# jing2li/MGPreconditionedGCR

Hardware: AMD Instinct MI355X
Metric: gcr_iterations_per_sec (higher is better)
Workload: dtype f64; 1 GPU; 3D 7-point Poisson 128^3 per GPU, unpreconditioned GCR restart 5, complex fp64, x0=0, RHS splitmix64 seed 0; rows=2097152, nnz=14581760, complex=True, stored_matrix_bytes=2097292, ell_width=7, tail_nnz=0, partition=1 GPU

## Files before the change

mgpreconditionedgcr_amd/csrc/gcr.hip:

```cpp
#include <climits>
#include <cmath>
#include <type_traits>

#include "internal.h"
#include "reduce.h"
#include "gcr_dev.h"
#include "pw_tail_dev.h"

namespace mgcr {

static EnvSwitch g_lean{"MGCR_LEAN"};
bool set_lean_enabled(bool on) { return g_lean.set(on); }

static double g_prof_phase_ms[3] = {0., 0., 0.};
static int g_prof_iters = 0;
static int g_prof_fused = 0;
void gcr_last_profile(double *phase_ms_total, int *n_iter, int *fused) {
    for (int k = 0; k < 3; k++) phase_ms_total[k] = g_prof_phase_ms[k];
    *n_iter = g_prof_iters;
    *fused = g_prof_fused;
}

struct GcrState {
    Op *A = nullptr;
// ... 1028 lines not shown
    s->r_after.clear();
    if (!p.left_precond && (!p.right_precond || pl.flex) && pl.max_it <= LND) s->r_after.assign((size_t)pl.max_it + 1, nullptr);
    return MGCR_OK;
}

struct Step {
    int it;
    bool tail;
    int lim;
    int ic_next;
    int nxt;
    const cplx *dir = nullptr;
    bool xr_now = false;
    const cplx *xr_in = nullptr;
    bool ended = false;
};

static int step_residual_lean(GcrState *s, const SolvePlan &pl, StepCursor &c, Step &st) {
    const int cur = c.cur;
    cplx *dslot = st.nxt >= 1 ? s->ps[st.nxt] : (pl.flex ? s->z : s->r);
    cplx *r_out = pl.flex ? s->r : dslot;
    const bool alpha_only = st.tail && pl.nested && !pl.multi;
    const bool deferred = alpha_only && s->defer_residual && !pl.flex && !s->r_after.empty();
    if (deferred || (alpha_only && s->discard_residual)) {
        KLAUNCH(alpha_only_kernel, 1, s->st, st.it, c.refA.p, c.refA.nblk, c.refA.stride, s->den + cur, cur, s->lc,
                deferred ? s->alphas + cur : (cplx *)nullptr);
        if (deferred) {
            s->defer_r_prev = c.rcur; s->defer_ap = s->aps[cur]; s->defer_alpha = s->alphas + cur; s->defer_it = c.global;
            s->r_after[(size_t)c.global] = c.rcur;
        } else {
            s->r_after.clear();
        }
        st.ended = true;
        return MGCR_OK;
    }
    st.xr_now = pl.xr_fuse && !st.tail;
    st.xr_in = c.rcur;
    if (c.xr_prefetched) c.xr_prefetched = false;
    else if (!st.xr_now)
        KLAUNCH((xr_update_kernel<true, true>), pl.g, s->st, st.it, c.refA.p, c.refA.nblk, c.refA.stride, (const cplx *)nullptr,
                (const cplx *)s->aps[cur], pl.x, c.rcur, r_out, pl.n, s->partsR, s->den + cur, s->alphas, cur, s->lc);
    c.rcur = r_out;
    st.dir = r_out;
    if (pl.flex && !st.tail) {
        MGCR_TRY(op_apply_raw((Op *)s->p.right_precond, s->r, dslot, pl.n));
        st.dir = dslot;
    }
    return MGCR_OK;
}

static int step_residual_classic(GcrState *s, const SolvePlan &pl, StepCursor &c, Step &st) {
    const mgcr_gcr_param &p = s->p;
    const int cur = c.cur;
// ... 34 lines not shown
static int step_one_launch(GcrState *s, const SolvePlan &pl, StepCursor &c, PhaseMarks &marks, const Step &st) {
    const int lim = st.lim;
    const bool closes = st.ic_next == 0;
    const cplx *vecs[FND], *cps[FND];
    for (int j = 0; j < FND; j++) { vecs[j] = s->aps[j < lim ? j : 0]; cps[j] = j < lim && j > 0 ? s->ps[j] : c.p0_live; }
    cplx *xr_out = nullptr;
    const bool next_is_special_last = c.global + 1 == pl.max_it && pl.nested && (s->defer_residual || s->discard_residual);
    if (c.global + 1 <= pl.max_it && !next_is_special_last && g_stepbuild_xr.on()) {
        const int ic2 = ((st.ic_next + 1) % s->restart == 0) ? 0 : st.ic_next + 1;
        const int nxt2 = ic2 % s->storage;
        MGCR_TRY(ensure_slot(s, nxt2));
        xr_out = nxt2 >= 1 ? s->ps[nxt2] : s->r;
    }
    MGCR_TRY(csr_step_build(pl.b0->csr, st.dir, pl.shift, pl.k, vecs, lim, s->st, st.it, c.refR.p, c.refR.nblk, c.refR.stride, s->hist,
                            s->hist_cap, s->den, s->aps[st.nxt], s->partsA, s->lc, pl.rmap, xr_out, s->den + st.nxt, st.nxt, s->partsR,
                            closes ? cps : nullptr, closes ? s->ps[0] : nullptr, closes ? pl.x : nullptr));
    c.xr_prefetched = xr_out != nullptr;
    marks.step_build = true;
    marks.step_build_xr = marks.step_build_xr || c.xr_prefetched;
    marks.step_build_close = marks.step_build_close || closes;
    if (closes) c.p0_live = s->ps[0];
    return MGCR_OK;
}

static int step_apply_dots(GcrState *s, const SolvePlan &pl, const StepCursor &c, const Step &st, bool *tail_rb) {
    const int lim = st.lim, nchunk = (lim + ND - 1) / ND;
    int ch0 = 0;
    if (pl.fuse_ok) {
        const int nf = lim < FND ? lim : FND;
        const cplx *vecs[FND];
        for (int j = 0; j < FND; j++) vecs[j] = s->aps[j < nf ? j : 0];
// ... 317 lines not shown
```

mgpreconditionedgcr_amd/csrc/gcr_dev.h:

```cpp
#pragma once
#include "internal.h"
#include "reduce.h"
#include "fused_form.h"

namespace mgcr {

constexpr int ND = 8;
constexpr int FND = 10;
constexpr int LND = 16;
#ifndef MGCR_NT_SLOTS
#define MGCR_NT_SLOTS 1
#endif
constexpr bool NTS = MGCR_NT_SLOTS != 0;

struct DevState {
    int stop_at;
    int base;
    int iter;
    int npend;
    double bnorm2;
    double rr;
    double tol2;
    int closed;
};
// ... 150 lines not shown
    }
    return c;
}

bool gcr_resident_eligible(const Op *A, const mgcr_gcr_param &p, int storage, int restart, int64_t n, bool lean, bool nested_handoff);
int gcr_resident_run(Op *A, const mgcr_gcr_param &p, int storage, int restart, const cplx *rhs, cplx *x, bool from_zero, bool alpha_only_last,
                     DevState *st, double *hist, int hist_cap, cplx *ring , SkipRef outer);

bool csr_step_build_eligible(const CsrDev &A, const DistCsr *dist, int lim);
bool csr_start_build_eligible(const CsrDev &A, const DistCsr *dist);
int csr_start_build(const CsrDev &A, const cplx *b, bool shift, cplx k, cplx *ap0, DevState *st, double *hist, LeanCoef *lc, cplx *den0,
                    cplx *r_out, double *partsR_out, const RowMap &rm);
int csr_step_build(const CsrDev &A, const cplx *x, bool shift, cplx k, const cplx *const *aps, int nd, DevState *st, int it, const double *partsR,
                   int nblkR, int strideR, double *hist, int hist_cap, const cplx *den, cplx *ap_out, double *partsA, LeanCoef *lc,
                   const RowMap &rm, cplx *xr_out = nullptr, cplx *xr_den_slot = nullptr, int xr_slot = 0, double *partsR_out = nullptr,
                   const cplx *const *close_ps = nullptr, cplx *close_p_out = nullptr, cplx *close_x = nullptr);

}
```

mgpreconditionedgcr_amd/csrc/gcr_stepbuild.hip:

```cpp
#include <climits>
#include <cstdlib>
#include <type_traits>

#include "internal.h"
#include "reduce.h"
#include "gcr_dev.h"
#include "spmv_dev.h"
#include "exchange_dev.h"

namespace mgcr {

constexpr int SB_MAX_TRIPS = 4;
constexpr int SB_MAX_ND = 5;
constexpr int SB_KEEP_TB = 2;
template <int NDT> constexpr int sb_keep_rows() { return NDT == 1 ? 3 : 2; }
template <int NDT, bool XR, bool CLOSE> constexpr bool sb_close_merged() { return CLOSE && (NDT == 4 || (NDT == 5 && XR)); }

struct StepBuildArgs {
    RowMat m;
    const cplx *x;
    const cplx *aps[SB_MAX_ND];
    int64_t n;
    int nlogical;
    RowMap rm;
    DevState *st;
    int it;
    const double *partsR;
    int nblkR, strideR;
    double *hist;
    int hist_cap;
    const cplx *den;
    cplx *ap_out;
    double *partsA;
    LeanCoef *lc;
    const cplx *ps[SB_MAX_ND];
    cplx *p_out;
    cplx *xvec;
    cplx *xr_out;
    cplx *xr_den_slot;
    int xr_slot;
    double *partsR_out;
    v4i *slots;
    unsigned gen0;
    unsigned *abort_dev;
    int *abort_host;
    int spin_limit;
    int test_stall;
};

__device__ __forceinline__ cplx sb_xr_alpha(const ResSync &sy, DevState *st, LeanCoef *lc, cplx *xr_den_slot, int xr_slot, int lb) {
    const cplx num = make_double2(res_total(sy, 0), res_total(sy, 1)), den = make_double2(res_total(sy, 2), res_total(sy, 3));
    const cplx alpha = to_sgpr(cdiv(num, den));
    if (lb == 0 && threadIdx.x == 0) {
        *xr_den_slot = den;
        st->npend = xr_slot + 1;
    }
    if (lb == 0 && (int)threadIdx.x < LND) lean_pending_update(lc, xr_slot, alpha, (int)threadIdx.x);
    return alpha;
}

template <int MODE, int WT, int NDT, bool XR, bool CLOSE, bool REALC = false>
__global__ void __launch_bounds__(RED_THREADS, 8) step_build_kernel(StepBuildArgs a) {
    __shared__ double lds[(2 * NDT > 4 ? 2 * NDT : 4) * 17];
    __shared__ double lds_pw[2 * SB_MAX_ND * 17], lds_ws[2 * SB_MAX_ND * RES_GRP];
    __shared__ int gave_up;
    __shared__ cplx sbeta[NDT], scp[NDT];
    extern __shared__ __attribute__((aligned(16))) unsigned char sb_smem[];
    if (a.st->stop_at < a.st->base + a.it) return;
    const int lb = logical_workgroup(a.rm, (int)blockIdx.x, (int)gridDim.x);
    if (lb >= a.nlogical) return;
    cplx *arL = reinterpret_cast<cplx *>(sb_smem);
    ResSync sy;
    res_sync_init(sy, a.slots, a.gen0, a.nlogical, lb, a.abort_dev, a.spin_limit, lds_pw, lds_ws, &gave_up);
    if (a.test_stall && lb == a.test_stall - 1) return;
    int64_t i0, end, stride;
    row_range(a.rm, lb, a.nlogical, a.n, &i0, &end, &stride);
    {
        double v[2 * NDT];
#pragma unroll
        for (int j = 0; j < 2 * NDT; j++) v[j] = 0.;
        int trip = 0;
        for (int64_t i = i0; i < end; i += stride, trip++) {
            const PatLds pl{nullptr, nullptr, nullptr};
            cplx sum;
            if constexpr (REALC) sum = sten_row_product_t<WT, false, 1>(a.m, i, [&](int32_t j) -> cplx { return a.x[j]; });
            else sum = fused_row_product<MODE, WT>(a.m, i, 0, pl, [&](int32_t j) -> cplx { return a.x[j]; });
            const cplx yi = a.m.shift ? csub(a.x[i], cmul(a.m.k, sum)) : sum;
            arL[trip * RED_THREADS + (int)threadIdx.x] = yi;
            __builtin_amdgcn_sched_barrier(0);
            cplx b[NDT];
#pragma unroll
            for (int j = 0; j < NDT; j++) b[j] = ld_stream<true>(a.aps[j] + i);
#pragma unroll
            for (int j = 0; j < NDT; j++) {
                cplx t = cconj_mul(yi, b[j]);
                v[2 * j] += t.x;
                v[2 * j + 1] += t.y;
            }
        }
        const double mine = block_sum_owner<2 * NDT>(v, lds);
        if ((int)threadIdx.x < 2 * NDT) {
            const v4i w4 = {__double2loint(mine), __double2hiint(mine), (int)sy.gen, 0};
            __builtin_amdgcn_raw_buffer_store_b128(w4, sy.slots, ((1 * RES_NV + (int)threadIdx.x) * RES_BLK + lb) * 16, 0, RES_SC1);
        }
    }
    constexpr bool PRE = NDT <= 3;
    cplx pre[NDT];
#pragma unroll
    for (int j = 0; j < NDT; j++) pre[j] = make_double2(0., 0.);
    if (PRE && i0 < end) {
#pragma unroll
        for (int j = 0; j < NDT; j++) pre[j] = ld_stream<NTS>((CLOSE ? a.ps[j] : a.aps[j]) + i0);
    }
    const bool ok = res_collect<2 * NDT>(sy, 1);
    if (!ok) {
        res_abort(a.abort_dev, a.abort_host);
        for (int64_t i = i0; i < end; i += stride) a.ap_out[i] = make_double2(__builtin_nan(""), __builtin_nan(""));
        if ((int)threadIdx.x < 4) a.partsA[threadIdx.x * RED_MAX_BLOCKS + lb] = __builtin_nan("");
        return;
    }
    bool ends_here = false;
    if (XR || lb == 0) {
        double rr[1];
        fold_partials<1>(a.partsR, a.nblkR, a.strideR, rr, lds);
        if (lb == 0 && threadIdx.x == 0) {
            close_step(a.st, a.it, rr[0], a.hist, a.hist_cap, CLOSE);
            if (CLOSE) a.st->closed = 1;
        }
        ends_here = !((rr[0] / a.st->bnorm2) > a.st->tol2);
    }
    if ((int)threadIdx.x < NDT) sbeta[threadIdx.x] = cdiv(make_double2(res_total(sy, 2 * threadIdx.x), res_total(sy, 2 * threadIdx.x + 1)), a.den[threadIdx.x]);
    __syncthreads();
    if constexpr (CLOSE) {
        if ((int)threadIdx.x < NDT) scp[threadIdx.x] = lean_close_coef(a.lc, sbeta, NDT, (int)threadIdx.x);
        __syncthreads();
    }
    if (!CLOSE && lb == 0 && (int)threadIdx.x <= NDT) lean_table_row<NDT>(a.lc, sbeta, (int)threadIdx.x);
    cplx beta[NDT];
#pragma unroll
    for (int j = 0; j < NDT; j++) beta[j] = to_sgpr(sbeta[j]);
    double v[4] = {0., 0., 0., 0.};
    int trip = 0;
    constexpr bool MERGED = sb_close_merged<NDT, XR, CLOSE>();
    cplx mcp[MERGED ? NDT : 1], mcx[MERGED ? NDT : 1];
    if constexpr (MERGED) {
#pragma unroll
        for (int j = 0; j < NDT; j++) {
            mcp[j] = to_sgpr(scp[j]);
            mcx[j] = to_sgpr(a.lc->cx[j]);
        }
    }
    auto close_row = [&](int64_t i, cplx dv) {
        cplx pj[NDT];
#pragma unroll
        for (int j = 0; j < NDT; j++) pj[j] = ld_stream<NTS>(a.ps[j] + i);
        cplx xv = a.xvec[i];
#pragma unroll
        for (int j = 0; j < NDT; j++) xv = cadd(xv, cmul(mcx[MERGED ? j : 0], pj[j]));
        a.xvec[i] = xv;
        cplx pc = make_double2(0., 0.);
#pragma unroll
        for (int j = 0; j < NDT; j++) pc = csub(pc, cmul(mcp[MERGED ? j : 0], pj[j]));
        st_stream<NTS>(a.p_out + i, cadd(dv, pc));
    };
    if constexpr (CLOSE && !MERGED) {
        cplx cp[NDT], cx[NDT];
#pragma unroll
        for (int j = 0; j < NDT; j++) {
            cp[j] = to_sgpr(scp[j]);
            cx[j] = to_sgpr(a.lc->cx[j]);
        }
        for (int64_t i = i0; i < end; i += stride) {
            cplx pj[NDT];
#pragma unroll
            for (int j = 0; j < NDT; j++) pj[j] = (PRE && i == i0) ? pre[j] : ld_stream<NTS>(a.ps[j] + i);
            const cplx dv = a.x[i];
            cplx xv = a.xvec[i];
#pragma unroll
            for (int j = 0; j < NDT; j++) xv = cadd(xv, cmul(cx[j], pj[j]));
            a.xvec[i] = xv;
            cplx pc = make_double2(0., 0.);
#pragma unroll
            for (int j = 0; j < NDT; j++) pc = csub(pc, cmul(cp[j], pj[j]));
            st_stream<NTS>(a.p_out + i, cadd(dv, pc));
        }
// ... 15 lines not shown
        cplx u = cconj_mul(an, an);
        v[2] += u.x; v[3] += u.y;
        return rv;
    };
    if constexpr (MERGED) {
        for (int64_t i = i0; i < end; i += stride, trip++) {
            const cplx rv = a.x[i];
            if (!XR || i + stride < end) close_row(i, rv);
            __builtin_amdgcn_sched_barrier(0);
            (void)build_row(i, trip, rv);
            __builtin_amdgcn_sched_barrier(0);
        }
    } else {
        for (int64_t i = i0; i < end; i += stride, trip++) (void)build_row(i, trip, make_double2(0., 0.));
    }
    const double mine = block_sum_owner<4>(v, lds);
    if (threadIdx.x < 4) a.partsA[threadIdx.x * RED_MAX_BLOCKS + lb] = mine;
    auto close_last = [&]() {
        if (trip > 0) {
            const int64_t il = i0 + (int64_t)(trip - 1) * stride;
            close_row(il, a.x[il]);
        }
        __builtin_amdgcn_sched_barrier(0);
    };
    if constexpr (XR) {
        if ((int)threadIdx.x < 4) {
            const v4i w4 = {__double2loint(mine), __double2hiint(mine), (int)sy.gen, 0};
            __builtin_amdgcn_raw_buffer_store_b128(w4, sy.slots, ((2 * RES_NV + (int)threadIdx.x) * RES_BLK + lb) * 16, 0, RES_SC1);
        }
        if constexpr (MERGED) close_last();
        const cplx xr0 = i0 < end ? a.x[i0] : make_double2(0., 0.);
        if (!res_collect<4>(sy, 2)) {
            res_abort(a.abort_dev, a.abort_host);
            for (int64_t i = i0; i < end; i += stride) a.xr_out[i] = make_double2(__builtin_nan(""), __builtin_nan(""));
            if (threadIdx.x == 0) a.partsR_out[lb] = __builtin_nan("");
            return;
        }
        if (ends_here) return;
        const cplx alpha = sb_xr_alpha(sy, a.st, a.lc, a.xr_den_slot, a.xr_slot, lb);
        double vr[1] = {0.};
        trip = 0;
        for (int64_t i = i0; i < end; i += stride, trip++) {
            const cplx rn = csub(i == i0 ? xr0 : a.x[i], cmul(alpha, arL[trip * RED_THREADS + (int)threadIdx.x]));
            a.xr_out[i] = rn;
            vr[0] += rn.x * rn.x + rn.y * rn.y;
        }
        const double tot = block_sum_owner<1>(vr, lds);
        if (threadIdx.x == 0) a.partsR_out[lb] = tot;
    }
}

template <class T>
__device__ __forceinline__ T *sb_elem(T *p, uint32_t off) {
    using C = std::conditional_t<std::is_const_v<T>, const char, char>;
    return reinterpret_cast<T *>(reinterpret_cast<C *>(p) + off);
}

__device__ __forceinline__ void sb_wave_pair_to_lds(double (&v)[2], double *lds, int k0) {
    double s;
    const int k = wave_multi_sum<2>(v, s);
    if (((int)threadIdx.x & 31) == 0) lds[(k0 + k) * 17 + ((int)threadIdx.x >> 6)] = s;
}
template <int NV>
__device__ __forceinline__ double sb_block_owner_from_lds(double *lds) {
    const int nwave = (blockDim.x + 63) >> 6;
    __syncthreads();
    double t = 0.;
    if (threadIdx.x < NV)
        for (int w = 0; w < nwave; w++) t += lds[threadIdx.x * 17 + w];
    return t;
}

template <int NDT, bool XR, bool CLOSE, bool REALC>
__global__ void __launch_bounds__(RED_THREADS, 8) step_keep_kernel(StepBuildArgs a) {
    __shared__ double lds[(2 * NDT > 4 ? 2 * NDT : 4) * 17];
    __shared__ double lds_pw[2 * SB_MAX_ND * 17], lds_ws[2 * SB_MAX_ND * RES_GRP];
    __shared__ int gave_up;
    __shared__ cplx sbeta[NDT], scp[NDT], scx[NDT];
    extern __shared__ __attribute__((aligned(16))) unsigned char sb_smem[];
    if (a.st->stop_at < a.st->base + a.it) return;
    const int lb = logical_workgroup(a.rm, (int)blockIdx.x, (int)gridDim.x);
    if (lb >= a.nlogical) return;
    cplx *arL = reinterpret_cast<cplx *>(sb_smem);
    const int tid = (int)threadIdx.x;
    ResSync sy;
    res_sync_init(sy, a.slots, a.gen0, a.nlogical, lb, a.abort_dev, a.spin_limit, lds_pw, lds_ws, &gave_up);
    if (a.test_stall && lb == a.test_stall - 1) return;
    int64_t i0, end, stride;
    row_range(a.rm, lb, a.nlogical, a.n, &i0, &end, &stride);
    auto row = [&](int t) -> int64_t { return i0 + (int64_t)t * stride; };
    uint32_t off[SB_MAX_TRIPS];
#pragma unroll
    for (int t = 0; t < SB_MAX_TRIPS; t++) off[t] = (uint32_t)row(t) * (uint32_t)sizeof(cplx);
    auto at = [&](auto *p, int t) { return sb_elem(p, off[t]); };
    cplx rk[SB_MAX_TRIPS];
#pragma unroll
    for (int t = 0; t < SB_MAX_TRIPS; t++) {
        const int64_t i = row(t);
        rk[t] = make_double2(0., 0.);
        if (i < end) {
            const PatLds pl{nullptr, nullptr, nullptr};
            cplx sum;
            const auto xj = [&](int32_t j) -> cplx { return *sb_elem(a.x, (uint32_t)j * (uint32_t)sizeof(cplx)); };
            if constexpr (REALC) sum = sten_row_product_t<7, false, 1>(a.m, i, xj);
            else sum = fused_row_product<3, 7>(a.m, i, 0, pl, xj);
            rk[t] = *at(a.x, t);
            arL[t * RED_THREADS + tid] = a.m.shift ? csub(rk[t], cmul(a.m.k, sum)) : sum;
        }
        __builtin_amdgcn_sched_barrier(0);
    }
// ... 10 lines not shown
#pragma unroll
            for (int t = 0; t < SB_MAX_TRIPS; t++) {
                if (row(t) < end) {
                    const cplx tt = cconj_mul(arL[t * RED_THREADS + tid], b[t]);
                    v[0] += tt.x;
                    v[1] += tt.y;
                }
            }
            if (j == 0) {
#pragma unroll
                for (int u = 0; u < KT; u++) pre[u] = b[u];
            }
            sb_wave_pair_to_lds(v, lds, 2 * j);
            __builtin_amdgcn_sched_barrier(0);
        }
        const double mine = sb_block_owner_from_lds<2 * NDT>(lds);
        if (tid < 2 * NDT) {
            const v4i w4 = {__double2loint(mine), __double2hiint(mine), (int)sy.gen, 0};
            __builtin_amdgcn_raw_buffer_store_b128(w4, sy.slots, ((1 * RES_NV + tid) * RES_BLK + lb) * 16, 0, RES_SC1);
        }
    }
    if (!res_collect<2 * NDT>(sy, 1)) {
        res_abort(a.abort_dev, a.abort_host);
        for (int64_t i = i0; i < end; i += stride) a.ap_out[i] = make_double2(__builtin_nan(""), __builtin_nan(""));
        if (tid < 4) a.partsA[tid * RED_MAX_BLOCKS + lb] = __builtin_nan("");
        return;
    }
    bool ends_here = false;
    if (XR || lb == 0) {
        double rr[1];
        fold_partials<1>(a.partsR, a.nblkR, a.strideR, rr, lds);
        if (lb == 0 && threadIdx.x == 0) {
            close_step(a.st, a.it, rr[0], a.hist, a.hist_cap, CLOSE);
            if (CLOSE) a.st->closed = 1;
        }
        ends_here = __builtin_amdgcn_readfirstlane(!((rr[0] / a.st->bnorm2) > a.st->tol2)) != 0;
    }
    if (tid < NDT) sbeta[tid] = cdiv(make_double2(res_total(sy, 2 * tid), res_total(sy, 2 * tid + 1)), a.den[tid]);
    __syncthreads();
    if constexpr (CLOSE) {
        if (tid < NDT) {
            scp[tid] = lean_close_coef(a.lc, sbeta, NDT, tid);
            scx[tid] = a.lc->cx[tid];
        }
        __syncthreads();
    }
    if (!CLOSE && lb == 0 && tid <= NDT) lean_table_row<NDT>(a.lc, sbeta, tid);
    {
        cplx beta[NDT];
#pragma unroll
        for (int j = 0; j < NDT; j++) beta[j] = to_sgpr(sbeta[j]);
        double v[4] = {0., 0., 0., 0.};
#pragma unroll
        for (int t0 = 0; t0 < SB_MAX_TRIPS; t0 += SB_KEEP_TB) {
            cplx ac[SB_KEEP_TB];
#pragma unroll
            for (int u = 0; u < SB_KEEP_TB; u++) ac[u] = make_double2(0., 0.);
#pragma unroll
            for (int j = 0; j < NDT; j++) {
                cplx aj[SB_KEEP_TB];
#pragma unroll
                for (int u = 0; u < SB_KEEP_TB; u++)
                    aj[u] = (j == 0 && t0 + u < KT) ? pre[t0 + u < KT ? t0 + u : 0]
                            : row(t0 + u) < end   ? ld_stream<NTS>(at(a.aps[j], t0 + u))
                                                  : make_double2(0., 0.);
#pragma unroll
                for (int u = 0; u < SB_KEEP_TB; u++) ac[u] = csub(ac[u], cmul(beta[j], aj[u]));
// ... 2 lines not shown
#pragma unroll
            for (int u = 0; u < SB_KEEP_TB; u++) {
                const int t = t0 + u;
                const int64_t i = row(t);
                if (i < end) {
                    const cplx an = cadd(arL[t * RED_THREADS + tid], ac[u]);
                    *at(a.ap_out, t) = an;
                    if (XR) arL[t * RED_THREADS + tid] = an;
                    const cplx tt = cconj_mul(rk[t], an);
                    v[0] += tt.x; v[1] += tt.y;
                    const cplx w = cconj_mul(an, an);
                    v[2] += w.x; v[3] += w.y;
                }
            }
        }
        const double mine = block_sum_owner<4>(v, lds);
        if (tid < 4) a.partsA[tid * RED_MAX_BLOCKS + lb] = mine;
        if (XR && tid < 4) {
            const v4i w4 = {__double2loint(mine), __double2hiint(mine), (int)sy.gen, 0};
            __builtin_amdgcn_raw_buffer_store_b128(w4, sy.slots, ((2 * RES_NV + tid) * RES_BLK + lb) * 16, 0, RES_SC1);
        }
    }
    if constexpr (CLOSE) {
        cplx cx[NDT], cp[NDT];
#pragma unroll
        for (int j = 0; j < NDT; j++) {
            cx[j] = to_sgpr(scx[j]);
            cp[j] = to_sgpr(scp[j]);
        }
#pragma unroll
        for (int t0 = 0; t0 < SB_MAX_TRIPS; t0 += SB_KEEP_TB) {
            cplx xv[SB_KEEP_TB], pc[SB_KEEP_TB];
#pragma unroll
            for (int u = 0; u < SB_KEEP_TB; u++) {
                xv[u] = row(t0 + u) < end ? *at(a.xvec, t0 + u) : make_double2(0., 0.);
                pc[u] = make_double2(0., 0.);
            }
#pragma unroll
            for (int j = 0; j < NDT; j++) {
                cplx pj[SB_KEEP_TB];
#pragma unroll
                for (int u = 0; u < SB_KEEP_TB; u++) pj[u] = row(t0 + u) < end ? ld_stream<NTS>(at(a.ps[j], t0 + u)) : make_double2(0., 0.);
// ... 1 lines not shown
                for (int u = 0; u < SB_KEEP_TB; u++) {
                    xv[u] = cadd(xv[u], cmul(cx[j], pj[u]));
                    pc[u] = csub(pc[u], cmul(cp[j], pj[u]));
                }
            }
#pragma unroll
            for (int u = 0; u < SB_KEEP_TB; u++) {
                const int64_t i = row(t0 + u);
                if (i < end) {
                    *at(a.xvec, t0 + u) = xv[u];
                    st_stream<NTS>(at(a.p_out, t0 + u), cadd(rk[t0 + u], pc[u]));
                }
            }
            __builtin_amdgcn_sched_barrier(0);
        }
    }
    if constexpr (XR) {
        if (!res_collect<4>(sy, 2)) {
            res_abort(a.abort_dev, a.abort_host);
            for (int64_t i = i0; i < end; i += stride) a.xr_out[i] = make_double2(__builtin_nan(""), __builtin_nan(""));
            if (threadIdx.x == 0) a.partsR_out[lb] = __builtin_nan("");
            return;
        }
        if (ends_here) return;
        const cplx alpha = sb_xr_alpha(sy, a.st, a.lc, a.xr_den_slot, a.xr_slot, lb);
        double vr[1] = {0.};
#pragma unroll
        for (int t = 0; t < SB_MAX_TRIPS; t++) {
            const int64_t i = row(t);
            if (i < end) {
                const cplx rn = csub(rk[t], cmul(alpha, arL[t * RED_THREADS + tid]));
                *at(a.xr_out, t) = rn;
                vr[0] += rn.x * rn.x + rn.y * rn.y;
            }
        }
        const double tot = block_sum_owner<1>(vr, lds);
        if (threadIdx.x == 0) a.partsR_out[lb] = tot;
    }
}

struct StartArgs {
    RowMat m;
    const cplx *b;
    cplx *ap0;
    int64_t n;
    int nlogical;
    RowMap rm;
    DevState *st;
    double *hist;
    LeanCoef *lc;
    cplx *den0;
    cplx *r_out;
// ... 50 lines not shown
        }
    }
    const cplx b0 = i0 < end ? a.b[i0] : make_double2(0., 0.);
    if (!res_collect<5>(sy, 1)) {
        res_abort(a.abort_dev, a.abort_host);
        for (int64_t i = i0; i < end; i += stride) a.r_out[i] = make_double2(__builtin_nan(""), __builtin_nan(""));
        if (threadIdx.x == 0) a.partsR_out[lb] = __builtin_nan("");
        return;
    }
    if (lb == 0 && threadIdx.x == 0) {
        const double nb = res_total(sy, 4);
        a.st->bnorm2 = nb;
        a.st->rr = nb;
        a.hist[0] = sqrt(nb) / sqrt(nb);
    }
    const cplx alpha = sb_xr_alpha(sy, a.st, a.lc, a.den0, 0, lb);
    double vr[1] = {0.};
#pragma unroll
    for (int t = 0; t < SB_MAX_TRIPS; t++) {
        const int64_t i = i0 + (int64_t)t * stride;
        if (i < end) {
            const cplx rn = csub(t == 0 ? b0 : a.b[i], cmul(alpha, apL[t * RED_THREADS + (int)threadIdx.x]));
            a.r_out[i] = rn;
            vr[0] += rn.x * rn.x + rn.y * rn.y;
        }
    }
    const double tot = block_sum_owner<1>(vr, lds);
    if (threadIdx.x == 0) a.partsR_out[lb] = tot;
}

static EnvSwitch g_stepbuild{"MGCR_STEPBUILD"}, g_start_build{"MGCR_START_BUILD"};
static EnvSwitch g_sb_keep_all{"MGCR_SB_KEEP_ALL"};
static EnvSwitch g_sb_real{"MGCR_SB_REAL"};
bool stepbuild_is_enabled() { return g_stepbuild.on(); }
bool set_stepbuild_enabled(bool on) { return g_stepbuild.set(on); }
bool set_start_build_enabled(bool on) { return g_start_build.set(on); }
bool set_stepbuild_keep_all_enabled(bool on) { return g_sb_keep_all.set(on); }
static int64_t g_stepbuild_launches = 0;
int64_t stepbuild_launch_count() { return g_stepbuild_launches; }

template <int NDT, bool XR, bool CLOSE> constexpr bool sb_keep_fits() { return NDT <= 2 || (NDT == 3 && !(XR && CLOSE)); }
template <int NDT, bool XR, bool CLOSE, bool R> const void *sb_keep() {
    if constexpr (sb_keep_fits<NDT, XR, CLOSE>()) return (const void *)step_keep_kernel<NDT, XR, CLOSE, R>;
    else return nullptr;
}
static const void *sb_kernel(int nd, bool xr, bool close, bool realc) {
    if (g_sb_keep_all.on() && nd <= 3) {
#define SKR(NDT, R) (close ? (xr ? sb_keep<NDT, true, true, R>() : sb_keep<NDT, false, true, R>()) \
                           : (xr ? sb_keep<NDT, true, false, R>() : sb_keep<NDT, false, false, R>()))
#define SKK(NDT) (realc ? SKR(NDT, true) : SKR(NDT, false))
        const void *keep = nd == 1 ? SKK(1) : nd == 2 ? SKK(2) : SKK(3);
#undef SKK
#undef SKR
        if (keep) return keep;
// ... 64 lines not shown
    a.test_stall = getenv("MGCR_TEST_STEPBUILD_STALL") ? atoi(getenv("MGCR_TEST_STEPBUILD_STALL")) : 0;
    a.spin_limit = getenv("MGCR_TEST_RESIDENT_SPIN_LIMIT") ? atoi(getenv("MGCR_TEST_RESIDENT_SPIN_LIMIT")) : RES_SPIN_LIMIT;
    return MGCR_OK;
}
static int sb_launch(const void *kernel, void *args, int grid, size_t lds_bytes, const char *who) {
    MGCR_CHECK(launch_is_coresident(kernel, RED_THREADS, lds_bytes, grid), MGCR_ERR_INVALID, "%s: launch would not be co-resident", who);
    void *kargs[1] = {args};
    MGCR_HIP(hipLaunchKernel(kernel, dim3((unsigned)grid), dim3(RED_THREADS), kargs, lds_bytes, ctx().stream));
    MGCR_HIP(hipGetLastError());
    return MGCR_OK;
}

int csr_step_build(const CsrDev &A, const cplx *x, bool shift, cplx k, const cplx *const *aps, int nd, DevState *st, int it, const double *partsR,
                   int nblkR, int strideR, double *hist, int hist_cap, const cplx *den, cplx *ap_out, double *partsA, LeanCoef *lc,
                   const RowMap &rm, cplx *xr_out, cplx *xr_den_slot, int xr_slot, double *partsR_out, const cplx *const *close_ps, cplx *close_p_out,
                   cplx *close_x) {
    MGCR_CHECK(nd >= 1 && nd <= SB_MAX_ND, MGCR_ERR_INVALID, "csr_step_build: 1..5 directions");
    StepBuildArgs a;
    MGCR_TRY(sb_fill_common(a, A, shift, k, st, rm, 3));
    a.x = x;
    for (int j = 0; j < SB_MAX_ND; j++) a.aps[j] = aps[j < nd ? j : 0];
    a.it = it; a.partsR = partsR; a.nblkR = nblkR; a.strideR = strideR; a.hist = hist; a.hist_cap = hist_cap;
    a.den = den; a.ap_out = ap_out; a.partsA = partsA; a.lc = lc;
    for (int j = 0; j < SB_MAX_ND; j++) a.ps[j] = close_ps ? close_ps[j < nd ? j : 0] : nullptr;
    a.p_out = close_p_out; a.xvec = close_x;
    a.xr_out = xr_out; a.xr_den_slot = xr_den_slot; a.xr_slot = xr_slot; a.partsR_out = partsR_out;
    MGCR_TRY(sb_launch(sb_kernel(nd, xr_out != nullptr, close_ps != nullptr, g_sb_real.on() && a.m.realv), &a, a.nlogical, sb_lds_bytes(A, a.nlogical),
                       "csr_step_build"));
    g_stepbuild_launches++;
    return MGCR_OK;
}

static int64_t g_start_build_launches = 0;
int64_t start_build_launch_count() { return g_start_build_launches; }
static const void *start_kernel(bool realc) {
    return realc ? (const void *)start_build_kernel<true> : (const void *)start_build_kernel<false>;
}

bool csr_start_build_eligible(const CsrDev &A, const DistCsr *dist) {
    if (!g_start_build.on() || !csr_step_build_eligible(A, dist, 1)) return false;
    const bool realc = g_sb_real.on() && row_mat(A, false, cplx{0., 0.}).realv;
    return launch_is_coresident(start_kernel(realc), RED_THREADS, sb_lds_bytes(A, red_grid(A.nrow)), red_grid(A.nrow));
}
// ... 15 lines not shown
```

Before: 14260 it/s.

## Ride residual-norm partials on the step-build grid exchange and stage coefficients in LDS

```diff
diff --git a/mgpreconditionedgcr_amd/csrc/gcr.hip b/mgpreconditionedgcr_amd/csrc/gcr.hip
--- a/mgpreconditionedgcr_amd/csrc/gcr.hip
+++ b/mgpreconditionedgcr_amd/csrc/gcr.hip
@@ -1066,6 +1066,7 @@
     bool xr_now = false;
     const cplx *xr_in = nullptr;
     bool ended = false;
+    bool r_one_launch = false;
 };
 
 static int step_residual_lean(GcrState *s, const SolvePlan &pl, StepCursor &c, Step &st) {
@@ -1088,7 +1089,7 @@
     }
     st.xr_now = pl.xr_fuse && !st.tail;
     st.xr_in = c.rcur;
-    if (c.xr_prefetched) c.xr_prefetched = false;
+    if (c.xr_prefetched) { c.xr_prefetched = false; st.r_one_launch = true; }
     else if (!st.xr_now)
         KLAUNCH((xr_update_kernel<true, true>), pl.g, s->st, st.it, c.refA.p, c.refA.nblk, c.refA.stride, (const cplx *)nullptr,
                 (const cplx *)s->aps[cur], pl.x, c.rcur, r_out, pl.n, s->partsR, s->den + cur, s->alphas, cur, s->lc);
@@ -1153,7 +1154,7 @@
     }
     MGCR_TRY(csr_step_build(pl.b0->csr, st.dir, pl.shift, pl.k, vecs, lim, s->st, st.it, c.refR.p, c.refR.nblk, c.refR.stride, s->hist,
                             s->hist_cap, s->den, s->aps[st.nxt], s->partsA, s->lc, pl.rmap, xr_out, s->den + st.nxt, st.nxt, s->partsR,
-                            closes ? cps : nullptr, closes ? s->ps[0] : nullptr, closes ? pl.x : nullptr));
+                            closes ? cps : nullptr, closes ? s->ps[0] : nullptr, closes ? pl.x : nullptr, st.r_one_launch));
     c.xr_prefetched = xr_out != nullptr;
     marks.step_build = true;
     marks.step_build_xr = marks.step_build_xr || c.xr_prefetched;
diff --git a/mgpreconditionedgcr_amd/csrc/gcr_dev.h b/mgpreconditionedgcr_amd/csrc/gcr_dev.h
--- a/mgpreconditionedgcr_amd/csrc/gcr_dev.h
+++ b/mgpreconditionedgcr_amd/csrc/gcr_dev.h
@@ -188,6 +188,7 @@
 int csr_step_build(const CsrDev &A, const cplx *x, bool shift, cplx k, const cplx *const *aps, int nd, DevState *st, int it, const double *partsR,
                    int nblkR, int strideR, double *hist, int hist_cap, const cplx *den, cplx *ap_out, double *partsA, LeanCoef *lc,
                    const RowMap &rm, cplx *xr_out = nullptr, cplx *xr_den_slot = nullptr, int xr_slot = 0, double *partsR_out = nullptr,
-                   const cplx *const *close_ps = nullptr, cplx *close_p_out = nullptr, cplx *close_x = nullptr);
+                   const cplx *const *close_ps = nullptr, cplx *close_p_out = nullptr, cplx *close_x = nullptr,
+                   bool partsR_one_launch = false );
 
 }
diff --git a/mgpreconditionedgcr_amd/csrc/gcr_stepbuild.hip b/mgpreconditionedgcr_amd/csrc/gcr_stepbuild.hip
--- a/mgpreconditionedgcr_amd/csrc/gcr_stepbuild.hip
+++ b/mgpreconditionedgcr_amd/csrc/gcr_stepbuild.hip
@@ -27,6 +27,7 @@
     int it;
     const double *partsR;
     int nblkR, strideR;
+    int ride;
     double *hist;
     int hist_cap;
     const cplx *den;
@@ -46,33 +47,86 @@
     int *abort_host;
     int spin_limit;
     int test_stall;
+#ifdef MGCR_SB_TIMING
+    unsigned long long *tick;
+#endif
 };
 
-__device__ __forceinline__ cplx sb_xr_alpha(const ResSync &sy, DevState *st, LeanCoef *lc, cplx *xr_den_slot, int xr_slot, int lb) {
+enum { SB_T_ENTRY, SB_T_GATHER, SB_T_PASS1, SB_T_PUB1, SB_T_COL1, SB_T_STREAM2, SB_T_PASS2, SB_T_PUB2, SB_T_COL2, SB_T_LAST, SB_TICKS };
+#ifdef MGCR_SB_TIMING
+#define SB_TICK(a, lb, p)                                                                        \
+    do {                                                                                         \
+        __builtin_amdgcn_sched_barrier(0);                                                       \
+        if ((a).tick && threadIdx.x == 0) (a).tick[(size_t)(lb) * SB_TICKS + (p)] = wall_clock64(); \
+        __builtin_amdgcn_sched_barrier(0);                                                       \
+    } while (0)
+#else
+#define SB_TICK(a, lb, p) do { } while (0)
+#endif
+
+__device__ __forceinline__ cplx sb_xr_alpha(const ResSync &sy) {
     const cplx num = make_double2(res_total(sy, 0), res_total(sy, 1)), den = make_double2(res_total(sy, 2), res_total(sy, 3));
-    const cplx alpha = to_sgpr(cdiv(num, den));
-    if (lb == 0 && threadIdx.x == 0) {
-        *xr_den_slot = den;
+    return to_sgpr(cdiv(num, den));
+}
+__device__ __forceinline__ void sb_xr_book(const ResSync &sy, DevState *st, LeanCoef *lc, cplx *xr_den_slot, int xr_slot, cplx alpha, int u) {
+    if (u == 0) {
+        *xr_den_slot = make_double2(res_total(sy, 2), res_total(sy, 3));
         st->npend = xr_slot + 1;
     }
-    if (lb == 0 && (int)threadIdx.x < LND) lean_pending_update(lc, xr_slot, alpha, (int)threadIdx.x);
-    return alpha;
+    if (u >= 0 && u < LND) lean_pending_update(lc, xr_slot, alpha, u);
+}
+
+template <int NDT>
+struct SbStage {
+    cplx den[NDT], cx[NDT];
+    double rpart;
+    double bnorm2, tol2;
+    double rr;
+    int ends;
+};
+template <int NDT, bool CLOSE>
+__device__ __forceinline__ void sb_stage_in(const StepBuildArgs &a, int lb, SbStage<NDT> &sg, LeanCoef *slc) {
+    static_assert(2 * NDT + NDT * NDT <= 64, "one staging wave");
+    const int tid = (int)threadIdx.x;
+    if (tid == RED_THREADS - 128 && a.ride) sg.rpart = a.partsR[lb];
+    if (tid == 64) {
+        sg.bnorm2 = a.st->bnorm2;
+        sg.tol2 = a.st->tol2;
+    }
+    if (tid < NDT) sg.den[tid] = a.den[tid];
+    if constexpr (CLOSE) {
+        const int w = tid - (RED_THREADS - 256);
+        const cplx *src = nullptr;
+        cplx *dst = nullptr;
+        if (w >= 0 && w < NDT) { src = a.lc->cx + w; dst = sg.cx + w; }
+        if (w >= NDT && w < 2 * NDT) { src = a.lc->t + (w - NDT); dst = slc->t + (w - NDT); }
+        if (w >= 2 * NDT && w < 2 * NDT + NDT * NDT) {
+            const int e = w - 2 * NDT, j = e / NDT, m = e - j * NDT;
+            src = a.lc->T + (j * LND + m); dst = slc->T + (j * LND + m);
+        }
+        if (src) *dst = *src;
+    }
 }
 
 template <int MODE, int WT, int NDT, bool XR, bool CLOSE, bool REALC = false>
 __global__ void __launch_bounds__(RED_THREADS, 8) step_build_kernel(StepBuildArgs a) {
     __shared__ double lds[(2 * NDT > 4 ? 2 * NDT : 4) * 17];
-    __shared__ double lds_pw[2 * SB_MAX_ND * 17], lds_ws[2 * SB_MAX_ND * RES_GRP];
+    __shared__ double lds_pw[2 * SB_MAX_ND * 17], lds_ws[(2 * SB_MAX_ND + 1) * RES_GRP];
     __shared__ int gave_up;
     __shared__ cplx sbeta[NDT], scp[NDT];
+    __shared__ SbStage<NDT> sg;
+    __shared__ cplx slc_mem[CLOSE ? sizeof(LeanCoef) / sizeof(cplx) : 1];
     extern __shared__ __attribute__((aligned(16))) unsigned char sb_smem[];
     if (a.st->stop_at < a.st->base + a.it) return;
     const int lb = logical_workgroup(a.rm, (int)blockIdx.x, (int)gridDim.x);
     if (lb >= a.nlogical) return;
     cplx *arL = reinterpret_cast<cplx *>(sb_smem);
+    LeanCoef *slc = reinterpret_cast<LeanCoef *>(slc_mem);
     ResSync sy;
     res_sync_init(sy, a.slots, a.gen0, a.nlogical, lb, a.abort_dev, a.spin_limit, lds_pw, lds_ws, &gave_up);
     if (a.test_stall && lb == a.test_stall - 1) return;
+    SB_TICK(a, lb, SB_T_ENTRY);
+    sb_stage_in<NDT, CLOSE>(a, lb, sg, slc);
     int64_t i0, end, stride;
     row_range(a.rm, lb, a.nlogical, a.n, &i0, &end, &stride);
     {
@@ -80,6 +134,7 @@
 #pragma unroll
         for (int j = 0; j < 2 * NDT; j++) v[j] = 0.;
         int trip = 0;
+        SB_TICK(a, lb, SB_T_GATHER);
         for (int64_t i = i0; i < end; i += stride, trip++) {
             const PatLds pl{nullptr, nullptr, nullptr};
             cplx sum;
@@ -98,11 +153,14 @@
                 v[2 * j + 1] += t.y;
             }
         }
-        const double mine = block_sum_owner<2 * NDT>(v, lds);
-        if ((int)threadIdx.x < 2 * NDT) {
+        SB_TICK(a, lb, SB_T_PASS1);
+        double mine = block_sum_owner<2 * NDT>(v, lds);
+        if ((int)threadIdx.x == 2 * NDT) mine = a.ride ? sg.rpart : 0.;
+        if ((int)threadIdx.x <= 2 * NDT) {
             const v4i w4 = {__double2loint(mine), __double2hiint(mine), (int)sy.gen, 0};
             __builtin_amdgcn_raw_buffer_store_b128(w4, sy.slots, ((1 * RES_NV + (int)threadIdx.x) * RES_BLK + lb) * 16, 0, RES_SC1);
         }
+        SB_TICK(a, lb, SB_T_PUB1);
     }
     constexpr bool PRE = NDT <= 3;
     cplx pre[NDT];
@@ -112,42 +170,51 @@
 #pragma unroll
         for (int j = 0; j < NDT; j++) pre[j] = ld_stream<NTS>((CLOSE ? a.ps[j] : a.aps[j]) + i0);
     }
-    const bool ok = res_collect<2 * NDT>(sy, 1);
+    const bool ok = res_collect<2 * NDT + 1>(sy, 1);
     if (!ok) {
         res_abort(a.abort_dev, a.abort_host);
         for (int64_t i = i0; i < end; i += stride) a.ap_out[i] = make_double2(__builtin_nan(""), __builtin_nan(""));
         if ((int)threadIdx.x < 4) a.partsA[threadIdx.x * RED_MAX_BLOCKS + lb] = __builtin_nan("");
         return;
     }
-    bool ends_here = false;
-    if (XR || lb == 0) {
-        double rr[1];
-        fold_partials<1>(a.partsR, a.nblkR, a.strideR, rr, lds);
-        if (lb == 0 && threadIdx.x == 0) {
-            close_step(a.st, a.it, rr[0], a.hist, a.hist_cap, CLOSE);
-            if (CLOSE) a.st->closed = 1;
-        }
-        ends_here = !((rr[0] / a.st->bnorm2) > a.st->tol2);
-    }
-    if ((int)threadIdx.x < NDT) sbeta[threadIdx.x] = cdiv(make_double2(res_total(sy, 2 * threadIdx.x), res_total(sy, 2 * threadIdx.x + 1)), a.den[threadIdx.x]);
+    SB_TICK(a, lb, SB_T_COL1);
+    if (XR || lb == a.nlogical - 1) {
+        double rr[1] = {0.};
+        if (!a.ride) fold_partials<1>(a.partsR, a.nblkR, a.strideR, rr, lds);
+        if (threadIdx.x == 64) {
+            if (a.ride) rr[0] = res_total(sy, 2 * NDT);
+            sg.rr = rr[0];
+            sg.ends = !((rr[0] / sg.bnorm2) > sg.tol2);
+        }
+    }
+    if ((int)threadIdx.x < NDT) sbeta[threadIdx.x] = cdiv(make_double2(res_total(sy, 2 * threadIdx.x), res_total(sy, 2 * threadIdx.x + 1)), sg.den[threadIdx.x]);
     __syncthreads();
     if constexpr (CLOSE) {
-        if ((int)threadIdx.x < NDT) scp[threadIdx.x] = lean_close_coef(a.lc, sbeta, NDT, (int)threadIdx.x);
+        if ((int)threadIdx.x < NDT) scp[threadIdx.x] = lean_close_coef(slc, sbeta, NDT, (int)threadIdx.x);
         __syncthreads();
     }
-    if (!CLOSE && lb == 0 && (int)threadIdx.x <= NDT) lean_table_row<NDT>(a.lc, sbeta, (int)threadIdx.x);
+    auto book = [&]() {
+        const int u = (int)threadIdx.x;
+        if (lb != a.nlogical - 1) return;
+        if (u == 0) {
+            close_step(a.st, a.it, sg.rr, a.hist, a.hist_cap, CLOSE);
+            if (CLOSE) a.st->closed = 1;
+        }
+        if (!CLOSE && u <= NDT) lean_table_row<NDT>(a.lc, sbeta, u);
+    };
     cplx beta[NDT];
 #pragma unroll
     for (int j = 0; j < NDT; j++) beta[j] = to_sgpr(sbeta[j]);
     double v[4] = {0., 0., 0., 0.};
     int trip = 0;
+    SB_TICK(a, lb, SB_T_STREAM2);
     constexpr bool MERGED = sb_close_merged<NDT, XR, CLOSE>();
     cplx mcp[MERGED ? NDT : 1], mcx[MERGED ? NDT : 1];
     if constexpr (MERGED) {
 #pragma unroll
         for (int j = 0; j < NDT; j++) {
             mcp[j] = to_sgpr(scp[j]);
-            mcx[j] = to_sgpr(a.lc->cx[j]);
+            mcx[j] = to_sgpr(sg.cx[j]);
         }
     }
     auto close_row = [&](int64_t i, cplx dv) {
@@ -168,7 +235,7 @@
 #pragma unroll
         for (int j = 0; j < NDT; j++) {
             cp[j] = to_sgpr(scp[j]);
-            cx[j] = to_sgpr(a.lc->cx[j]);
+            cx[j] = to_sgpr(sg.cx[j]);
         }
         for (int64_t i = i0; i < end; i += stride) {
             cplx pj[NDT];
@@ -214,8 +281,11 @@
     } else {
         for (int64_t i = i0; i < end; i += stride, trip++) (void)build_row(i, trip, make_double2(0., 0.));
     }
+    SB_TICK(a, lb, SB_T_PASS2);
     const double mine = block_sum_owner<4>(v, lds);
     if (threadIdx.x < 4) a.partsA[threadIdx.x * RED_MAX_BLOCKS + lb] = mine;
+    if (!XR) book();
+    if (!XR) SB_TICK(a, lb, SB_T_LAST);
     auto close_last = [&]() {
         if (trip > 0) {
             const int64_t il = i0 + (int64_t)(trip - 1) * stride;
@@ -228,16 +298,19 @@
             const v4i w4 = {__double2loint(mine), __double2hiint(mine), (int)sy.gen, 0};
             __builtin_amdgcn_raw_buffer_store_b128(w4, sy.slots, ((2 * RES_NV + (int)threadIdx.x) * RES_BLK + lb) * 16, 0, RES_SC1);
         }
+        SB_TICK(a, lb, SB_T_PUB2);
         if constexpr (MERGED) close_last();
         const cplx xr0 = i0 < end ? a.x[i0] : make_double2(0., 0.);
+        book();
         if (!res_collect<4>(sy, 2)) {
             res_abort(a.abort_dev, a.abort_host);
             for (int64_t i = i0; i < end; i += stride) a.xr_out[i] = make_double2(__builtin_nan(""), __builtin_nan(""));
             if (threadIdx.x == 0) a.partsR_out[lb] = __builtin_nan("");
             return;
         }
-        if (ends_here) return;
-        const cplx alpha = sb_xr_alpha(sy, a.st, a.lc, a.xr_den_slot, a.xr_slot, lb);
+        SB_TICK(a, lb, SB_T_COL2);
+        if (sg.ends) return;
+        const cplx alpha = sb_xr_alpha(sy);
         double vr[1] = {0.};
         trip = 0;
         for (int64_t i = i0; i < end; i += stride, trip++) {
@@ -245,8 +318,10 @@
             a.xr_out[i] = rn;
             vr[0] += rn.x * rn.x + rn.y * rn.y;
         }
+        if (lb == a.nlogical - 1) sb_xr_book(sy, a.st, a.lc, a.xr_den_slot, a.xr_slot, sb_xr_alpha(sy), (int)threadIdx.x);
         const double tot = block_sum_owner<1>(vr, lds);
         if (threadIdx.x == 0) a.partsR_out[lb] = tot;
+        SB_TICK(a, lb, SB_T_LAST);
     }
 }
 
@@ -274,18 +349,23 @@
 template <int NDT, bool XR, bool CLOSE, bool REALC>
 __global__ void __launch_bounds__(RED_THREADS, 8) step_keep_kernel(StepBuildArgs a) {
     __shared__ double lds[(2 * NDT > 4 ? 2 * NDT : 4) * 17];
-    __shared__ double lds_pw[2 * SB_MAX_ND * 17], lds_ws[2 * SB_MAX_ND * RES_GRP];
+    __shared__ double lds_pw[2 * SB_MAX_ND * 17], lds_ws[(2 * SB_MAX_ND + 1) * RES_GRP];
     __shared__ int gave_up;
-    __shared__ cplx sbeta[NDT], scp[NDT], scx[NDT];
+    __shared__ cplx sbeta[NDT], scp[NDT];
+    __shared__ SbStage<NDT> sg;
+    __shared__ cplx slc_mem[CLOSE ? sizeof(LeanCoef) / sizeof(cplx) : 1];
     extern __shared__ __attribute__((aligned(16))) unsigned char sb_smem[];
     if (a.st->stop_at < a.st->base + a.it) return;
     const int lb = logical_workgroup(a.rm, (int)blockIdx.x, (int)gridDim.x);
     if (lb >= a.nlogical) return;
     cplx *arL = reinterpret_cast<cplx *>(sb_smem);
+    LeanCoef *slc = reinterpret_cast<LeanCoef *>(slc_mem);
     const int tid = (int)threadIdx.x;
     ResSync sy;
     res_sync_init(sy, a.slots, a.gen0, a.nlogical, lb, a.abort_dev, a.spin_limit, lds_pw, lds_ws, &gave_up);
     if (a.test_stall && lb == a.test_stall - 1) return;
+    SB_TICK(a, lb, SB_T_ENTRY);
+    sb_stage_in<NDT, CLOSE>(a, lb, sg, slc);
     int64_t i0, end, stride;
     row_range(a.rm, lb, a.nlogical, a.n, &i0, &end, &stride);
     auto row = [&](int t) -> int64_t { return i0 + (int64_t)t * stride; };
@@ -294,6 +374,7 @@
     for (int t = 0; t < SB_MAX_TRIPS; t++) off[t] = (uint32_t)row(t) * (uint32_t)sizeof(cplx);
     auto at = [&](auto *p, int t) { return sb_elem(p, off[t]); };
     cplx rk[SB_MAX_TRIPS];
+    SB_TICK(a, lb, SB_T_GATHER);
 #pragma unroll
     for (int t = 0; t < SB_MAX_TRIPS; t++) {
         const int64_t i = row(t);
@@ -334,43 +415,52 @@
             sb_wave_pair_to_lds(v, lds, 2 * j);
             __builtin_amdgcn_sched_barrier(0);
         }
-        const double mine = sb_block_owner_from_lds<2 * NDT>(lds);
-        if (tid < 2 * NDT) {
+        SB_TICK(a, lb, SB_T_PASS1);
+        double mine = sb_block_owner_from_lds<2 * NDT>(lds);
+        if (tid == 2 * NDT) mine = a.ride ? sg.rpart : 0.;
+        if (tid <= 2 * NDT) {
             const v4i w4 = {__double2loint(mine), __double2hiint(mine), (int)sy.gen, 0};
             __builtin_amdgcn_raw_buffer_store_b128(w4, sy.slots, ((1 * RES_NV + tid) * RES_BLK + lb) * 16, 0, RES_SC1);
         }
-    }
-    if (!res_collect<2 * NDT>(sy, 1)) {
+        SB_TICK(a, lb, SB_T_PUB1);
+    }
+    if (!res_collect<2 * NDT + 1>(sy, 1)) {
         res_abort(a.abort_dev, a.abort_host);
         for (int64_t i = i0; i < end; i += stride) a.ap_out[i] = make_double2(__builtin_nan(""), __builtin_nan(""));
         if (tid < 4) a.partsA[tid * RED_MAX_BLOCKS + lb] = __builtin_nan("");
         return;
     }
-    bool ends_here = false;
-    if (XR || lb == 0) {
-        double rr[1];
-        fold_partials<1>(a.partsR, a.nblkR, a.strideR, rr, lds);
-        if (lb == 0 && threadIdx.x == 0) {
-            close_step(a.st, a.it, rr[0], a.hist, a.hist_cap, CLOSE);
-            if (CLOSE) a.st->closed = 1;
-        }
-        ends_here = __builtin_amdgcn_readfirstlane(!((rr[0] / a.st->bnorm2) > a.st->tol2)) != 0;
-    }
-    if (tid < NDT) sbeta[tid] = cdiv(make_double2(res_total(sy, 2 * tid), res_total(sy, 2 * tid + 1)), a.den[tid]);
+    SB_TICK(a, lb, SB_T_COL1);
+    if (XR || lb == a.nlogical - 1) {
+        double rr[1] = {0.};
+        if (!a.ride) fold_partials<1>(a.partsR, a.nblkR, a.strideR, rr, lds);
+        if (tid == 64) {
+            if (a.ride) rr[0] = res_total(sy, 2 * NDT);
+            sg.rr = rr[0];
+            sg.ends = !((rr[0] / sg.bnorm2) > sg.tol2);
+        }
+    }
+    if (tid < NDT) sbeta[tid] = cdiv(make_double2(res_total(sy, 2 * tid), res_total(sy, 2 * tid + 1)), sg.den[tid]);
     __syncthreads();
     if constexpr (CLOSE) {
-        if (tid < NDT) {
-            scp[tid] = lean_close_coef(a.lc, sbeta, NDT, tid);
-            scx[tid] = a.lc->cx[tid];
-        }
+        if (tid < NDT) scp[tid] = lean_close_coef(slc, sbeta, NDT, tid);
         __syncthreads();
     }
-    if (!CLOSE && lb == 0 && tid <= NDT) lean_table_row<NDT>(a.lc, sbeta, tid);
+    auto book = [&]() {
+        const int u = tid;
+        if (lb != a.nlogical - 1) return;
+        if (u == 0) {
+            close_step(a.st, a.it, sg.rr, a.hist, a.hist_cap, CLOSE);
+            if (CLOSE) a.st->closed = 1;
+        }
+        if (!CLOSE && u <= NDT) lean_table_row<NDT>(a.lc, sbeta, u);
+    };
     {
         cplx beta[NDT];
 #pragma unroll
         for (int j = 0; j < NDT; j++) beta[j] = to_sgpr(sbeta[j]);
         double v[4] = {0., 0., 0., 0.};
+        SB_TICK(a, lb, SB_T_STREAM2);
 #pragma unroll
         for (int t0 = 0; t0 < SB_MAX_TRIPS; t0 += SB_KEEP_TB) {
             cplx ac[SB_KEEP_TB];
@@ -403,18 +493,20 @@
                 }
             }
         }
+        SB_TICK(a, lb, SB_T_PASS2);
         const double mine = block_sum_owner<4>(v, lds);
         if (tid < 4) a.partsA[tid * RED_MAX_BLOCKS + lb] = mine;
         if (XR && tid < 4) {
             const v4i w4 = {__double2loint(mine), __double2hiint(mine), (int)sy.gen, 0};
             __builtin_amdgcn_raw_buffer_store_b128(w4, sy.slots, ((2 * RES_NV + tid) * RES_BLK + lb) * 16, 0, RES_SC1);
         }
+        SB_TICK(a, lb, XR ? SB_T_PUB2 : SB_T_LAST);
     }
     if constexpr (CLOSE) {
         cplx cx[NDT], cp[NDT];
 #pragma unroll
         for (int j = 0; j < NDT; j++) {
-            cx[j] = to_sgpr(scx[j]);
+            cx[j] = to_sgpr(sg.cx[j]);
             cp[j] = to_sgpr(scp[j]);
         }
 #pragma unroll
@@ -446,7 +538,9 @@
             }
             __builtin_amdgcn_sched_barrier(0);
         }
-    }
+        if (!XR) SB_TICK(a, lb, SB_T_LAST);
+    }
+    book();
     if constexpr (XR) {
         if (!res_collect<4>(sy, 2)) {
             res_abort(a.abort_dev, a.abort_host);
@@ -454,8 +548,9 @@
             if (threadIdx.x == 0) a.partsR_out[lb] = __builtin_nan("");
             return;
         }
-        if (ends_here) return;
-        const cplx alpha = sb_xr_alpha(sy, a.st, a.lc, a.xr_den_slot, a.xr_slot, lb);
+        SB_TICK(a, lb, SB_T_COL2);
+        if (sg.ends) return;
+        const cplx alpha = sb_xr_alpha(sy);
         double vr[1] = {0.};
 #pragma unroll
         for (int t = 0; t < SB_MAX_TRIPS; t++) {
@@ -466,8 +561,10 @@
                 vr[0] += rn.x * rn.x + rn.y * rn.y;
             }
         }
+        if (lb == a.nlogical - 1) sb_xr_book(sy, a.st, a.lc, a.xr_den_slot, a.xr_slot, sb_xr_alpha(sy), tid);
         const double tot = block_sum_owner<1>(vr, lds);
         if (threadIdx.x == 0) a.partsR_out[lb] = tot;
+        SB_TICK(a, lb, SB_T_LAST);
     }
 }
 
@@ -548,7 +645,8 @@
         a.st->rr = nb;
         a.hist[0] = sqrt(nb) / sqrt(nb);
     }
-    const cplx alpha = sb_xr_alpha(sy, a.st, a.lc, a.den0, 0, lb);
+    const cplx alpha = sb_xr_alpha(sy);
+    if (lb == 0) sb_xr_book(sy, a.st, a.lc, a.den0, 0, alpha, (int)threadIdx.x);
     double vr[1] = {0.};
 #pragma unroll
     for (int t = 0; t < SB_MAX_TRIPS; t++) {
@@ -572,6 +670,45 @@
 bool set_stepbuild_keep_all_enabled(bool on) { return g_sb_keep_all.set(on); }
 static int64_t g_stepbuild_launches = 0;
 int64_t stepbuild_launch_count() { return g_stepbuild_launches; }
+
+#ifdef MGCR_SB_TIMING
+constexpr int SB_TIMING_CAP = 64;
+struct SbTimingRec { int nd, xr, close, keep, nlogical; };
+static unsigned long long *g_sb_tick = nullptr;
+static SbTimingRec g_sb_tick_rec[SB_TIMING_CAP];
+static int64_t g_sb_tick_count = 0;
+static unsigned long long *sb_timing_slot(int nd, bool xr, bool close, bool keep, int nlogical) {
+    static const bool on = getenv("MGCR_SB_TIMING") && atoi(getenv("MGCR_SB_TIMING")) != 0;
+    if (!on) return nullptr;
+    const size_t per = (size_t)RES_BLK * SB_TICKS;
+    if (!g_sb_tick && hipMalloc((void **)&g_sb_tick, SB_TIMING_CAP * per * sizeof(unsigned long long)) != hipSuccess) { (void)hipGetLastError(); return nullptr; }
+    const int slot = (int)(g_sb_tick_count++ % SB_TIMING_CAP);
+    g_sb_tick_rec[slot] = SbTimingRec{nd, xr, close, keep, nlogical};
+    if (hipMemsetAsync(g_sb_tick + slot * per, 0, per * sizeof(unsigned long long), ctx().stream) != hipSuccess) { (void)hipGetLastError(); return nullptr; }
+    return g_sb_tick + slot * per;
+}
+extern "C" int mgcr_sb_timing_dump(const char *path) {
+    if (!g_sb_tick) return MGCR_ERR_INVALID;
+    const size_t per = (size_t)RES_BLK * SB_TICKS;
+    std::vector<unsigned long long> h(SB_TIMING_CAP * per);
+    if (hipDeviceSynchronize() != hipSuccess || hipMemcpy(h.data(), g_sb_tick, h.size() * sizeof(unsigned long long), hipMemcpyDeviceToHost) != hipSuccess) return MGCR_ERR_HIP;
+    FILE *f = fopen(path, "w");
+    if (!f) return MGCR_ERR_INVALID;
+    const int64_t first = g_sb_tick_count > SB_TIMING_CAP ? g_sb_tick_count - SB_TIMING_CAP : 0;
+    for (int64_t l = first; l < g_sb_tick_count; l++) {
+        const int slot = (int)(l % SB_TIMING_CAP);
+        const SbTimingRec &r = g_sb_tick_rec[slot];
+        for (int b = 0; b < r.nlogical; b++) {
+            fprintf(f, "%lld %d %d %d %d %d", (long long)l, r.nd, r.xr, r.close, r.keep, b);
+            for (int q = 0; q < SB_TICKS; q++) fprintf(f, " %llu", h[slot * per + (size_t)b * SB_TICKS + q]);
+            fprintf(f, "\n");
+        }
+    }
+    fclose(f);
+    g_sb_tick_count = 0;
+    return MGCR_OK;
+}
+#endif
 
 template <int NDT, bool XR, bool CLOSE> constexpr bool sb_keep_fits() { return NDT <= 2 || (NDT == 3 && !(XR && CLOSE)); }
 template <int NDT, bool XR, bool CLOSE, bool R> const void *sb_keep() {
@@ -666,19 +803,23 @@
 int csr_step_build(const CsrDev &A, const cplx *x, bool shift, cplx k, const cplx *const *aps, int nd, DevState *st, int it, const double *partsR,
                    int nblkR, int strideR, double *hist, int hist_cap, const cplx *den, cplx *ap_out, double *partsA, LeanCoef *lc,
                    const RowMap &rm, cplx *xr_out, cplx *xr_den_slot, int xr_slot, double *partsR_out, const cplx *const *close_ps, cplx *close_p_out,
-                   cplx *close_x) {
+                   cplx *close_x, bool partsR_one_launch) {
     MGCR_CHECK(nd >= 1 && nd <= SB_MAX_ND, MGCR_ERR_INVALID, "csr_step_build: 1..5 directions");
     StepBuildArgs a;
     MGCR_TRY(sb_fill_common(a, A, shift, k, st, rm, 3));
     a.x = x;
     for (int j = 0; j < SB_MAX_ND; j++) a.aps[j] = aps[j < nd ? j : 0];
     a.it = it; a.partsR = partsR; a.nblkR = nblkR; a.strideR = strideR; a.hist = hist; a.hist_cap = hist_cap;
+    a.ride = partsR_one_launch && nblkR == a.nlogical && nblkR > 1;
     a.den = den; a.ap_out = ap_out; a.partsA = partsA; a.lc = lc;
     for (int j = 0; j < SB_MAX_ND; j++) a.ps[j] = close_ps ? close_ps[j < nd ? j : 0] : nullptr;
     a.p_out = close_p_out; a.xvec = close_x;
     a.xr_out = xr_out; a.xr_den_slot = xr_den_slot; a.xr_slot = xr_slot; a.partsR_out = partsR_out;
-    MGCR_TRY(sb_launch(sb_kernel(nd, xr_out != nullptr, close_ps != nullptr, g_sb_real.on() && a.m.realv), &a, a.nlogical, sb_lds_bytes(A, a.nlogical),
-                       "csr_step_build"));
+    const void *kernel = sb_kernel(nd, xr_out != nullptr, close_ps != nullptr, g_sb_real.on() && a.m.realv);
+#ifdef MGCR_SB_TIMING
+    a.tick = sb_timing_slot(nd, xr_out != nullptr, close_ps != nullptr, g_sb_keep_all.on() && nd <= 3 && !(nd == 3 && xr_out && close_ps), a.nlogical);
+#endif
+    MGCR_TRY(sb_launch(kernel, &a, a.nlogical, sb_lds_bytes(A, a.nlogical), "csr_step_build"));
     g_stepbuild_launches++;
     return MGCR_OK;
 }
```

Measured after the change: 14130 it/s. About the same (-0.9%).
